# hermanjakobsen/robotic-ultrasound-imaging

Hardware: AMD Instinct MI355X
Metric: env-steps/sec (whole node) at 4096 envs/GPU, random-action rollout (higher is better)
Workload: dtype f32

## Files before the change

### robotic-ultrasound-imaging_amd/csrc/usim_step16.h

```cpp
#pragma once
#include <type_traits>

namespace usim {

template <int N, class F>
DI void static_for(F&& f) {
    if constexpr (N > 0) { static_for<N - 1>(f); f(std::integral_constant<int, N - 1>{}); }
}

template <int CTRL>
DI float dpp0(float v) { return __int_as_float(__builtin_amdgcn_update_dpp(0, __float_as_int(v), CTRL, 0xf, 0xf, true)); }
template <int G> DI int glane() { return (int)(threadIdx.x & (G - 1)); }
template <int G, int K> DI float rbc(float v) {
    if constexpr (G == 16) return dpp0<0x150 + K>(v);
    else {
        const int iv = __float_as_int(v);
        const int t = __builtin_amdgcn_update_dpp(iv, iv, 0x150 + K, 0xf, 0x3, false);
        return __int_as_float(__builtin_amdgcn_update_dpp(t, iv, 0x150 + 8 + K, 0xf, 0xc, false));
    }
}
template <int G, int D> DI float rshr0(float v) {
    const float t = dpp0<0x110 + D>(v);
    if constexpr (G == 16) return t; else return (glane<G>() < D) ? 0.f : t;
}
template <int G, int D> DI float rshl0(float v) {
    const float t = dpp0<0x100 + D>(v);
    if constexpr (G == 16) return t; else return (glane<G>() >= G - D) ? 0.f : t;
}
template <int G, int D> DI float rshr(float v, float fill) {
    const float t = __int_as_float(__builtin_amdgcn_update_dpp(__float_as_int(fill), __float_as_int(v), 0x110 + D, 0xf, 0xf, false));
    if constexpr (G == 16) return t; else return (glane<G>() < D) ? fill : t;
}
template <int K> DI float qbc(float v) { return dpp0<K * 0x55>(v); }
template <int G, int K> DI f3 rbc3(f3 v) { return mk(rbc<G, K>(v.x), rbc<G, K>(v.y), rbc<G, K>(v.z)); }
template <int G> DI float prefix_sum(float v) { v += rshr0<G, 1>(v); v += rshr0<G, 2>(v); v += rshr0<G, 4>(v); return v; }
template <int G> DI float suffix_sum(float v) { v += rshl0<G, 1>(v); v += rshl0<G, 2>(v); v += rshl0<G, 4>(v); return v; }
template <int G> DI f3 prefix_sum(f3 v) { return mk(prefix_sum<G>(v.x), prefix_sum<G>(v.y), prefix_sum<G>(v.z)); }
template <int G> DI f3 suffix_sum(f3 v) { return mk(suffix_sum<G>(v.x), suffix_sum<G>(v.y), suffix_sum<G>(v.z)); }

constexpr int TASK_LANE[6] = {0, 1, 2, 4, 5, 6};

#define USIM_DPP_BC(K) " row_newbcast:" #K " row_mask:0xf bank_mask:0xf\n\t"
#define USIM_DPP_LO(K) " row_newbcast:" #K " row_mask:0xf bank_mask:0x3\n\t"
DI float row_times_joint7(const float* A, float v) {
    float s;
    asm("s_nop 1\n\t"
        "v_mul_f32_dpp %0, %1, %2" USIM_DPP_BC(0) "v_fmac_f32_dpp %0, %1, %3" USIM_DPP_BC(1) "v_fmac_f32_dpp %0, %1, %4" USIM_DPP_BC(2)
        "v_fmac_f32_dpp %0, %1, %5" USIM_DPP_BC(3) "v_fmac_f32_dpp %0, %1, %6" USIM_DPP_BC(4) "v_fmac_f32_dpp %0, %1, %7" USIM_DPP_BC(5)
        "v_fmac_f32_dpp %0, %1, %8" USIM_DPP_BC(6)
        : "=&v"(s) : "v"(v), "v"(A[0]), "v"(A[1]), "v"(A[2]), "v"(A[3]), "v"(A[4]), "v"(A[5]), "v"(A[6]));
    return s;
}
DI float row_times_joint7_g8(const float* A, float v) {
    float s;
    asm("s_nop 1\n\t"
        "v_mul_f32_dpp %0, %1, %2 row_newbcast:0 row_mask:0xf bank_mask:0x3\n\t"  "v_mul_f32_dpp %0, %1, %2 row_newbcast:8 row_mask:0xf bank_mask:0xc\n\t"
        "v_fmac_f32_dpp %0, %1, %3 row_newbcast:1 row_mask:0xf bank_mask:0x3\n\t" "v_fmac_f32_dpp %0, %1, %3 row_newbcast:9 row_mask:0xf bank_mask:0xc\n\t"
        "v_fmac_f32_dpp %0, %1, %4 row_newbcast:2 row_mask:0xf bank_mask:0x3\n\t" "v_fmac_f32_dpp %0, %1, %4 row_newbcast:10 row_mask:0xf bank_mask:0xc\n\t"
        "v_fmac_f32_dpp %0, %1, %5 row_newbcast:3 row_mask:0xf bank_mask:0x3\n\t" "v_fmac_f32_dpp %0, %1, %5 row_newbcast:11 row_mask:0xf bank_mask:0xc\n\t"
        "v_fmac_f32_dpp %0, %1, %6 row_newbcast:4 row_mask:0xf bank_mask:0x3\n\t" "v_fmac_f32_dpp %0, %1, %6 row_newbcast:12 row_mask:0xf bank_mask:0xc\n\t"
        "v_fmac_f32_dpp %0, %1, %7 row_newbcast:5 row_mask:0xf bank_mask:0x3\n\t" "v_fmac_f32_dpp %0, %1, %7 row_newbcast:13 row_mask:0xf bank_mask:0xc\n\t"
        "v_fmac_f32_dpp %0, %1, %8 row_newbcast:6 row_mask:0xf bank_mask:0x3\n\t" "v_fmac_f32_dpp %0, %1, %8 row_newbcast:14 row_mask:0xf bank_mask:0xc"
        : "=&v"(s) : "v"(v), "v"(A[0]), "v"(A[1]), "v"(A[2]), "v"(A[3]), "v"(A[4]), "v"(A[5]), "v"(A[6]));
    return s;
}
template <int G, int NJ_>
DI float row_times_joint(const float* A, float v) {
    static_assert(NJ_ == 7, "seven joint lanes");
    if constexpr (G == 16) return row_times_joint7(A, v); else return row_times_joint7_g8(A, v);
}
template <int G>
DI float col_times_task(const float* A, float t) {
    float s;
    if constexpr (G == 16) {
        asm("s_nop 1\n\t"
            "v_mul_f32_dpp %0, %1, %2" USIM_DPP_BC(0) "v_fmac_f32_dpp %0, %1, %3" USIM_DPP_BC(1) "v_fmac_f32_dpp %0, %1, %4" USIM_DPP_BC(2)
            "v_fmac_f32_dpp %0, %1, %5" USIM_DPP_BC(4) "v_fmac_f32_dpp %0, %1, %6" USIM_DPP_BC(5) "v_fmac_f32_dpp %0, %1, %7" USIM_DPP_BC(6)
            : "=&v"(s) : "v"(t), "v"(A[0]), "v"(A[1]), "v"(A[2]), "v"(A[3]), "v"(A[4]), "v"(A[5]));
    } else {
        asm("s_nop 1\n\t"
            "v_mul_f32_dpp %0, %1, %2 row_newbcast:0 row_mask:0xf bank_mask:0x3\n\t"  "v_mul_f32_dpp %0, %1, %2 row_newbcast:8 row_mask:0xf bank_mask:0xc\n\t"
            "v_fmac_f32_dpp %0, %1, %3 row_newbcast:1 row_mask:0xf bank_mask:0x3\n\t" "v_fmac_f32_dpp %0, %1, %3 row_newbcast:9 row_mask:0xf bank_mask:0xc\n\t"
            "v_fmac_f32_dpp %0, %1, %4 row_newbcast:2 row_mask:0xf bank_mask:0x3\n\t" "v_fmac_f32_dpp %0, %1, %4 row_newbcast:10 row_mask:0xf bank_mask:0xc\n\t"
            "v_fmac_f32_dpp %0, %1, %5 row_newbcast:4 row_mask:0xf bank_mask:0x3\n\t" "v_fmac_f32_dpp %0, %1, %5 row_newbcast:12 row_mask:0xf bank_mask:0xc\n\t"
            "v_fmac_f32_dpp %0, %1, %6 row_newbcast:5 row_mask:0xf bank_mask:0x3\n\t" "v_fmac_f32_dpp %0, %1, %6 row_newbcast:13 row_mask:0xf bank_mask:0xc\n\t"
            "v_fmac_f32_dpp %0, %1, %7 row_newbcast:6 row_mask:0xf bank_mask:0x3\n\t" "v_fmac_f32_dpp %0, %1, %7 row_newbcast:14 row_mask:0xf bank_mask:0xc"
            : "=&v"(s) : "v"(t), "v"(A[0]), "v"(A[1]), "v"(A[2]), "v"(A[3]), "v"(A[4]), "v"(A[5]));
    }
    return s;
}
template <int G, int K>
// ... 34 lines not shown
            "v_fmac_f32_dpp %0, %4, %10 row_newbcast:%13 row_mask:0xf bank_mask:0x3\n\t" "v_fmac_f32_dpp %0, %4, %10 row_newbcast:%14 row_mask:0xf bank_mask:0xc\n\t"
            "v_fmac_f32_dpp %0, %5, %11 row_newbcast:%13 row_mask:0xf bank_mask:0x3\n\t" "v_fmac_f32_dpp %0, %5, %11 row_newbcast:%14 row_mask:0xf bank_mask:0xc\n\t"
            "v_fmac_f32_dpp %0, %6, %12 row_newbcast:%13 row_mask:0xf bank_mask:0x3\n\t" "v_fmac_f32_dpp %0, %6, %12 row_newbcast:%14 row_mask:0xf bank_mask:0xc"
            : "=&v"(s) : "v"(z.x), "v"(z.y), "v"(z.z), "v"(vo.x), "v"(vo.y), "v"(vo.z), "v"(n.x), "v"(n.y), "v"(n.z), "v"(f.x), "v"(f.y), "v"(f.z), "n"(K), "n"(K + 8));
    }
    return s;
}

template <int G>
DI void fk16(const float* at, const float q, f3& X, f3& Y, f3& Z, f3& P) {
    float s, c;
    sincos_(q, s, c);
    const f3 f0 = mk(at[AT_RFIX], at[AT_RFIX + 1], at[AT_RFIX + 2]), f1 = mk(at[AT_RFIX + 3], at[AT_RFIX + 4], at[AT_RFIX + 5]);
    X = f0 * c + f1 * s; Y = f1 * c - f0 * s; Z = mk(at[AT_RFIX + 6], at[AT_RFIX + 7], at[AT_RFIX + 8]);
    P = mk(at[AT_LPOS], at[AT_LPOS + 1], at[AT_LPOS + 2]);
    static_for<3>([&](auto Dc) {
        constexpr int D = 1 << decltype(Dc)::value;
        const f3 LX = mk(rshr<G, D>(X.x, 1.f), rshr<G, D>(X.y, 0.f), rshr<G, D>(X.z, 0.f));
        const f3 LY = mk(rshr<G, D>(Y.x, 0.f), rshr<G, D>(Y.y, 1.f), rshr<G, D>(Y.z, 0.f));
        const f3 LZ = mk(rshr<G, D>(Z.x, 0.f), rshr<G, D>(Z.y, 0.f), rshr<G, D>(Z.z, 1.f));
        const f3 LP = mk(rshr0<G, D>(P.x), rshr0<G, D>(P.y), rshr0<G, D>(P.z));
        const f3 nX = LX * X.x + LY * X.y + LZ * X.z, nY = LX * Y.x + LY * Y.y + LZ * Y.z, nZ = LX * Z.x + LY * Z.y + LZ * Z.z;
        P = LP + LX * P.x + LY * P.y + LZ * P.z;
        X = nX; Y = nY; Z = nZ;
    });
}

DI void jacobian_rows(float* xl, const int gl, const float* Jc, float* Jr) {
    if (gl < 8) {
#pragma unroll
        for (int a = 0; a < 6; ++a) xl[a * 8 + gl] = Jc[a];
    }
    group_sync();
    int arow = (gl & 7) - ((gl & 4) ? 1 : 0);
    arow = arow > 5 ? 5 : arow;
    const float4 j0 = *reinterpret_cast<const float4*>(&xl[arow * 8]), j1 = *reinterpret_cast<const float4*>(&xl[arow * 8 + 4]);
    Jr[0] = j0.x; Jr[1] = j0.y; Jr[2] = j0.z; Jr[3] = j0.w; Jr[4] = j1.x; Jr[5] = j1.y; Jr[6] = j1.z; Jr[7] = j1.w;
}

template <int G>
DI float solve6_task(float* A, float b, const int gl) {
    static_for<6>([&](auto Kc) {
        constexpr int k = decltype(Kc)::value;
        constexpr int lk = TASK_LANE[k];
        const float g = (A[k] - (gl == lk ? 1.f : 0.f)) * rcp_(rbc<G, lk>(A[k]));
#pragma unroll
        for (int c = k + 1; c < 6; ++c) A[c] = fmaf(-g, rbc<G, lk>(A[c]), A[c]);
        b = fmaf(-g, rbc<G, lk>(b), b);
    });
    return b;
}

constexpr int X16_WORDS = 64;
constexpr int X16_RIGID_STRIDE = 84;

#ifndef USIM_WPR16
#define USIM_WPR16 4
#endif
#ifndef USIM_WPR8
#define USIM_WPR8 4
#endif
template <int G> constexpr int wpr() { return G == 16 ? USIM_WPR16 : USIM_WPR8; }
constexpr int MB_POSE = X16_WORDS;
constexpr int MB_OP = MB_POSE + 12;
constexpr int MB_W = MB_OP + 64;
constexpr int MB_Q = MB_W + 16;
constexpr int MB_GOAL = MB_Q + 100;
#ifndef USIM_DRAW_AHEAD
#define USIM_DRAW_AHEAD 1
#endif
constexpr bool DRAW_AHEAD = USIM_DRAW_AHEAD != 0;
#ifndef USIM_LIST_AHEAD
#define USIM_LIST_AHEAD 0
#endif
constexpr bool LIST_AHEAD = USIM_LIST_AHEAD != 0;
#ifndef USIM_LATTICE_AHEAD
#define USIM_LATTICE_AHEAD 1
#endif
constexpr bool LATTICE_AHEAD = USIM_LATTICE_AHEAD != 0;
#ifndef USIM_LATTICE_PRIO
#define USIM_LATTICE_PRIO 1
#endif
constexpr bool LATTICE_PRIO = USIM_LATTICE_PRIO != 0;
constexpr int MB_ACT = MB_GOAL + 12;
constexpr int X2_STRIDE = MB_ACT + (DRAW_AHEAD ? 8 : 0);
template <int G> constexpr int x2_base() { return TB_WORDS + (64 * wpr<G>() / G) * GE_STRIDE; }
static_assert(x2_base<16>() % 4 == 0 && x2_base<8>() % 4 == 0 && X2_STRIDE % 4 == 0 && MB_OP % 4 == 0 && MB_W % 4 == 0 && MB_ACT % 4 == 0, "mailbox block: 16-byte accesses");
static_assert((x2_base<8>() + 32 * X2_STRIDE) * 4 <= 160 * 1024, "split kernel with 8-lane groups: LDS of a CU");
#ifndef USIM_ARM_CULL16
#define USIM_ARM_CULL16 0
#endif
template <int G> constexpr int arm_cull_rounds() { return G == 16 ? USIM_ARM_CULL16 : 7; }
static_assert(!LATTICE_AHEAD || USIM_ARM_CULL16 == 0, "LATTICE_AHEAD: the arm wave must not need the integrated element positions (no broad-phase rounds on its side)");
template <int ROLE, int G, bool RES> constexpr bool lattice_ahead() { return LATTICE_AHEAD && ROLE != 0 && G == 16 && RES; }

#if defined(USIM_TSTAMP) || defined(USIM_TSTAMP_NOWAIT)
#define USIM_BAR() do { __syncthreads(); ++nbar; } while (0)
#else
#define USIM_BAR() __syncthreads()
#endif


constexpr int ARM_LDS_WORDS = A16_LANES * AT_STRIDE;
template <int TORSO, int ROLE, int G> constexpr int arm_lds_base();
template <int NE, class WR = NoWarm>
struct Carry {
    float dqj, qdj, q0j;
    Episode ep;
    float s[NE], sd[NE];
    WR wr;
};

template <int TORSO, int ROLE, int G> constexpr int arm_lds_base() {
    return ROLE != 0 ? x2_base<G>() + (64 * wpr<G>() / G) * X2_STRIDE : (TORSO ? SOFT16_LDS_WORDS : 16 * X16_RIGID_STRIDE);
}
static_assert((arm_lds_base<1, 1, 8>() + ARM_LDS_WORDS) * 4 <= 160 * 1024 && arm_lds_base<1, 1, 8>() % 4 == 0 && arm_lds_base<1, 1, 16>() % 4 == 0 && arm_lds_base<1, 0, 16>() % 4 == 0
              && arm_lds_base<0, 0, 16>() % 4 == 0, "arm table behind the LDS blocks of every 16-lane kernel");

template <int TORSO, int MODE, int ROLE, int NT, int G = 16, bool RES = false, class WR = NoWarm, bool AHEAD = false>
DI void step16_one(float* lds, const DevModel& M, const DevCfg& C, float* __restrict__ st, const int n, const int npad, const DevIO& io, const int flags, const long long rstep,
                   const bool first_pass, const int sub, const bool more, int& nbar, Carry<TORSO ? (N_TOP + G - 1) / G : 1, WR>& cy) {
    static_assert(!AHEAD || (ROLE == 1 && RES), "action drawn ahead: the arm wave of a resident split launch");
    constexpr bool WARM = !std::is_same<WR, NoWarm>::value;
    static_assert(!WARM || (TORSO == 1 && ROLE == 0) || (TORSO == 1 && MODE == 0), "warm start: the soft-torso kernels");
    constexpr int WPR = (ROLE != 0) ? wpr<G>() : 4;
    constexpr int EPW = 64 / G, EPB = WPR * EPW;
    static_assert(!RES || MODE == 0, "resident state: step launches only");
    constexpr int X2_BASE = x2_base<G>();
    constexpr unsigned GMASK = (G == 16) ? 0xffffu : 0xffu;
    static_assert(G == 16 || (TORSO == 1 && MODE == 0 && ROLE != 0), "8-lane groups: the split soft-torso step only");
    constexpr int NE = TORSO ? (N_TOP + G - 1) / G : 1;
    static_assert(ROLE == 0 || (TORSO == 1 && MODE == 0), "the split kernel is the soft-torso step");
    const int lane = threadIdx.x & 63, wave = (threadIdx.x >> 6) & (WPR - 1);
    constexpr bool LA = lattice_ahead<ROLE, G, RES>();
    constexpr bool RES_HERE = RES && (LA || !(ROLE == 2 && G == 16));
    const bool fresh = !RES_HERE || first_pass;
    const int gl = lane & (G - 1), ge = lane / G;
    const int gbase = lane - gl;
    const int eb = wave * EPW + ge;
    const bool auto_reset = (flags & LF_AUTO_RESET) != 0;
    unsigned long long* const dbg = io.dbg;
    const bool refill = (MODE == 1) && io.refill != 0;
    const int item_cnt = refill ? io.count[0] : 1;
    const int item_first = refill ? (int)blockIdx.x * EPB : 0;
    for (int item0 = item_first; item0 < item_cnt; item0 += refill ? (int)gridDim.x * EPB : 1) {
    int env = blockIdx.x * EPB + eb;
    bool valid = env < n;
    int item_ep = 0;
    if (refill) {
        valid = item0 + eb < item_cnt;
        const int2 it = valid ? io.items[item0 + eb] : make_int2(0, 0);
        env = it.x; item_ep = it.y;
    }
    const bool store = valid && gl == 0;
    const int ei = valid ? env : (refill ? 0 : n - 1);
#define LAT(w) st[(size_t)F_LAT * npad + (size_t)ei * LAT_ENV_WORDS + (w)]
#define EB(off) lds[TB_WORDS + eb * GE_STRIDE + (off)]
    float* const warm_rows = st + warm_index(io.bank_row0, npad, (size_t)ei);
    int mbo = X2_BASE + eb * X2_STRIDE;
    if constexpr (ROLE != 0) asm volatile("" : "+v"(mbo));
    float* const xl = (ROLE != 0) ? &lds[mbo]
                                  : (TORSO ? &lds[TB_WORDS + eb * GE_STRIDE + GE_WS] : &lds[eb * X16_RIGID_STRIDE]);
    static_assert(GE_WS + X16_WORDS <= GE_STRIDE, "transpose scratch overlays the wrench records");
    constexpr int GOAL_OFF = (ROLE != 0) ? MB_GOAL : (TORSO ? GE_CG + (MAXCAND + 1) * CG_WORDS - GE_WS : X16_WORDS);
    static_assert(GE_CG + (MAXCAND + 1) * CG_WORDS + 12 <= GE_STRIDE && X16_WORDS + 12 <= X16_RIGID_STRIDE, "room for the goal");
    float* const goal_lds = xl + GOAL_OFF;

    USIM_STAMP(dbg, 0);
    if constexpr (ROLE == 1) { if (dbg && blockIdx.x == 0 && threadIdx.x == 0) dbg[20] = __builtin_readcyclecounter(); }

    float at[AT_STRIDE];
    {
        constexpr int ARM_LDS = arm_lds_base<TORSO, ROLE, G>();
        const float4* ap = fresh ? reinterpret_cast<const float4*>(M.tables + TB_ARM + gl * AT_STRIDE) : reinterpret_cast<const float4*>(lds + ARM_LDS + gl * AT_STRIDE);
        if (fresh) {
#pragma unroll
            for (int v = 0; v < AT_STRIDE / 4; ++v) { const float4 x = ap[v]; at[4 * v] = x.x; at[4 * v + 1] = x.y; at[4 * v + 2] = x.z; at[4 * v + 3] = x.w; }
            if constexpr (RES && ROLE != 2) {
                if (lane < G) {
#pragma unroll
                    for (int v = 0; v < AT_STRIDE / 4; ++v) reinterpret_cast<float4*>(lds + ARM_LDS + gl * AT_STRIDE)[v] = make_float4(at[4 * v], at[4 * v + 1], at[4 * v + 2], at[4 * v + 3]);
                }
            }
        } else {
            const float4* lp = reinterpret_cast<const float4*>(lds + ARM_LDS + gl * AT_STRIDE);
#pragma unroll
            for (int v = 0; v < AT_STRIDE / 4; ++v) { const float4 x = lp[v]; at[4 * v] = x.x; at[4 * v + 1] = x.y; at[4 * v + 2] = x.z; at[4 * v + 3] = x.w; }
        }
    }
    const float* const sp = st + scalar_index(0, (size_t)ei);
    const bool jlane = at[AT_JOINT] != 0.f;
    const int jl = jlane ? gl : NJ - 1;
    float &dqj = cy.dqj, &qdj = cy.qdj, &q0j = cy.q0j;
    Episode& E = cy.ep;
    f3 &ts = E.ts, &te = E.te;
    float &u0 = E.u0, &vbar = E.vbar, &fzbar = E.fzbar, &fzprev = E.fzprev, &dfz = E.dfz, &kst = E.kst, &kdmp = E.kdmp, &mu = E.mu, &epret = E.epret;
    int &t = E.t, &touched = E.touched, &episode = E.episode, &status = E.status;
    float (&s_pre)[NE] = cy.s, (&sd_pre)[NE] = cy.sd;
    if (fresh) {
        dqj = sp[F_Q + jl]; qdj = sp[F_QD + jl]; q0j = sp[F_Q0 + jl];
        float sv[20];
        {
            const float4* s4 = reinterpret_cast<const float4*>(sp + 20);
#pragma unroll
            for (int v = 0; v < 5; ++v) { const float4 x = s4[v]; sv[4 * v] = x.x; sv[4 * v + 1] = x.y; sv[4 * v + 2] = x.z; sv[4 * v + 3] = x.w; }
        }
#define SV(f) sv[(f) - 20]
        ts = mk(SV(F_TS), SV(F_TS + 1), SV(F_TS + 2)); te = mk(SV(F_TE), SV(F_TE + 1), SV(F_TE + 2));
        u0 = SV(F_U0); vbar = SV(F_VBAR); fzbar = SV(F_FZBAR); fzprev = SV(F_FZPREV); dfz = SV(F_DFZ);
        kst = SV(F_KST); kdmp = SV(F_KDMP); mu = SV(F_MU); epret = SV(F_EPRET);
        t = __float_as_int(SV(F_T)); touched = __float_as_int(SV(F_TOUCH)); episode = __float_as_int(SV(F_EPISODE)); status = __float_as_int(SV(F_STATUS));
#undef SV
#pragma unroll
        for (int i = 0; i < NE; ++i) {
            const int e = gl + i * G;
            s_pre[i] = 0.f; sd_pre[i] = 0.f;
            if (TORSO && MODE == 0 && ROLE != 1 && e < N_TOP) { s_pre[i] = LAT(LAT_S + e); sd_pre[i] = LAT(LAT_SD + e); }
            if (TORSO && MODE == 0 && ROLE == 1 && !LA && e < N_TOP) s_pre[i] = LAT(LAT_S + e);
        }
        if constexpr (WARM && MODE == 0 && ROLE != 1) warm_load(warm_rows, gl, cy.wr);
    } else if constexpr (RES && ROLE == 1 && !LA) {
#pragma unroll
        for (int i = 0; i < NE; ++i) { const int e = gl + i * G; s_pre[i] = (e < N_TOP) ? EB(GE_S + e) : 0.f; }
    } else if constexpr (RES && ROLE == 2 && !LA) {
        const float4 nx = *reinterpret_cast<const float4*>(&lds[mbo + MB_W]);
        if (nx.w != 0.f) {
            kst = nx.x; kdmp = nx.y; mu = nx.z; t = 0;
#pragma unroll
            for (int i = 0; i < NE; ++i) { s_pre[i] = 0.f; sd_pre[i] = 0.f; }
            warm_clear(cy.wr);
        }
    }
    if (!jlane) { dqj = 0.f; qdj = 0.f; q0j = 0.f; }
    float qj = q0j + dqj;
    if (TORSO != 0 && item0 == item_first && first_pass) {
        const float4* src = reinterpret_cast<const float4*>(M.tables);
        float4* dst = reinterpret_cast<float4*>(lds);
        constexpr int NV = TB_WORDS / 4, PER = (NV + NT - 1) / NT;
        float4 tmp[PER];
        int tix = threadIdx.x;
        asm volatile("" : "+v"(tix));
#pragma unroll
        for (int i = 0; i < PER; ++i) { int idx = tix + i * NT; tmp[i] = (idx < NV) ? src[idx] : make_float4(0, 0, 0, 0); }
#pragma unroll
        for (int i = 0; i < PER; ++i) { int idx = tix + i * NT; if (idx < NV) dst[idx] = tmp[i]; }
        USIM_BAR();
    }
    USIM_STAMP(dbg, 1);

    if (MODE == 0 && sub == 0) t += 1;
    const bool last_sub = sub == C.substeps - 1;
    const int tphys = (MODE == 0) ? (t - 1) * C.substeps + sub : 0;
    const float dt = C.dt, inv_h = rcp_((float)C.horizon);
#if defined(USIM_TSTAMP) || defined(USIM_TSTAMP_NOWAIT)
#define RSTAMP(k) do { if (dbg && blockIdx.x == 0 && (threadIdx.x & (64 * WPR - 1)) == 0) dbg[(ROLE == 2 ? 30 : 20) + (k)] = __builtin_readcyclecounter(); } while (0)
#else
#define RSTAMP(k) do { } while (0)
#endif
#define XSTAMP(k) RSTAMP(20 + (k))
    if constexpr (ROLE == 2) {
        RSTAMP(0);
        if constexpr (LA && LATTICE_PRIO) __builtin_amdgcn_s_setprio(1);
        float* const mb = &lds[mbo];
        const int* tb_shell = reinterpret_cast<const int*>(lds + TB_SHELL);
        float dz, vz, az;
        torso_motion(C, tphys, dz, vz, az);
        if constexpr (LA) {
            if (first_pass) {
#pragma unroll
                for (int i = 0; i < NE; ++i) { const int e = gl + i * G; if (e < N_TOP) EB(GE_S + e) = s_pre[i]; }
            }
        }
        lattice_rhs<G, NE>(lds, eb, gl, M, az, kst, kdmp, true, s_pre, sd_pre);
        lattice_solve<G>(lds, eb, gl, gbase);
        RSTAMP(1);
        USIM_BAR();
        RSTAMP(2);
        if constexpr (LA && LATTICE_PRIO) __builtin_amdgcn_s_setprio(0);
        if constexpr (LA) {
            if (!first_pass) {
                const float4 nx = *reinterpret_cast<const float4*>(&mb[MB_W]);
                const bool began = nx.w != 0.f;
                if (__any(began)) {
                    if (began) {
                        kst = nx.x; kdmp = nx.y; mu = nx.z; t = 0;
                        if (sub == 0) t += 1;
#pragma unroll
                        for (int i = 0; i < NE; ++i) { const int e = gl + i * G; s_pre[i] = 0.f; sd_pre[i] = 0.f; if (e < N_TOP) EB(GE_S + e) = 0.f; }
                        warm_clear(cy.wr);
                    }
                    torso_motion(C, (t - 1) * C.substeps + sub, dz, vz, az);
                    lattice_rhs<G, NE>(lds, eb, gl, M, az, kst, kdmp, true, s_pre, sd_pre);
                    lattice_solve<G>(lds, eb, gl, gbase);
                }
            }
        }
        const f3 xs = mk(mb[MB_POSE], mb[MB_POSE + 1], mb[MB_POSE + 2]), sy = mk(mb[MB_POSE + 3], mb[MB_POSE + 4], mb[MB_POSE + 5]),
                 sz = mk(mb[MB_POSE + 6], mb[MB_POSE + 7], mb[MB_POSE + 8]);
        const f3 sxc = cross(sy, sz);
        int nq = __float_as_int(mb[MB_POSE + 10]);
#pragma unroll
        for (int i = arm_cull_rounds<G>(); i < NE; ++i) {
            const int eraw = i * G + gl, e = eraw < N_TOP ? eraw : N_TOP - 1;
            const bool cand = (eraw < N_TOP) && collide_cull(lds, e, M, C, s_pre[i], dz, xs, sxc, sz);
            const unsigned gm = (unsigned)(__ballot(cand) >> gbase) & GMASK;
            mb[MB_Q + (cand ? nq + __popc(gm & ((1u << gl) - 1u)) : 99)] = __int_as_float(e);
            nq += __popc(gm);
        }
        group_sync();
#if defined(USIM_TSTAMP) || defined(USIM_TSTAMP_NOWAIT)
        if (dbg && blockIdx.x == 0 && wave == 0 && gl == 0) dbg[54 + ge] = 1ull + (unsigned long long)nq;
#endif
        int nc = 0;
        collide_queue<G>(lds, mb + MB_Q, nq, &EB(GE_CG), gl, gbase, M, C, &EB(GE_S), dz, xs, sxc, sy, sz, nc);
        constexpr bool EARLY = G == 8;
        ContactRows P;
        constexpr bool LIST_EARLY = EARLY || (G == 16 && LIST_AHEAD);
        int nc_early = nc, overflow_early = 0, ncmax_early = 0, cel_early[MAXC];
        if constexpr (LIST_EARLY) {
            contact_overflow<G>(lds, eb, gl, gbase, nc_early);
            if (nc_early > MAXC) { overflow_early = 1; nc_early = MAXC; }
            group_sync();
            if constexpr (G == 16) {
                const int m01 = max(__builtin_amdgcn_readlane(nc_early, 0), __builtin_amdgcn_readlane(nc_early, 16));
                const int m23 = max(__builtin_amdgcn_readlane(nc_early, 32), __builtin_amdgcn_readlane(nc_early, 48));
                ncmax_early = max(m01, m23);
            } else {
#pragma unroll
                for (int k = MAXC; k >= 1; --k) if (ncmax_early == 0 && __any(nc_early >= k)) ncmax_early = k;
            }
#pragma unroll
            for (int k = 0; k < MAXC; ++k) cel_early[k] = (k < nc_early) ? __float_as_int(EB(GE_CG + k * CG_WORDS + 6)) : 0;
            if constexpr (EARLY) { if (ncmax_early > 0) contact_rows<G>(lds, eb, gl, M, C, nc_early, cel_early, vz, P); }
        }
        RSTAMP(3);
        USIM_BAR();
        RSTAMP(4);
        if constexpr (LA && LATTICE_PRIO) __builtin_amdgcn_s_setprio(1);
        if constexpr (!LIST_EARLY) contact_overflow<G>(lds, eb, gl, gbase, nc);
        int overflow = 0;
        if (nc > MAXC) { overflow = 1; nc = MAXC; }
        if constexpr (!LIST_EARLY) group_sync();
        XSTAMP(0);
        int ncmax = 0;
        if constexpr (LIST_EARLY) { nc = nc_early; overflow = overflow_early; ncmax = ncmax_early; }
        else {
#pragma unroll
            for (int k = MAXC; k >= 1; --k) if (ncmax == 0 && __any(nc >= k)) ncmax = k;
        }
        XSTAMP(1);
        float gf[MAXC], W[6] = {0, 0, 0, 0, 0, 0};
        int cel[MAXC];
#pragma unroll
        for (int k = 0; k < MAXC; ++k) { const int ek = __float_as_int(EB(GE_CG + k * CG_WORDS + 6)); gf[k] = 0.f; cel[k] = LIST_EARLY ? cel_early[k] : ((k < nc) ? ek : 0); }
        if (ncmax > 0) {
            float alpha[6], vs[6], Lp[21];
#pragma unroll
            for (int a = 0; a < 6; ++a) {
                alpha[a] = mb[MB_OP + 48 + a]; vs[a] = mb[MB_OP + 54 + a];
#pragma unroll
                for (int b = 0; b <= a; ++b) Lp[PK(a, b)] = mb[MB_OP + a * 8 + b];
            }
            XSTAMP(2);
            contact_solve<G, EARLY, true>(lds, eb, gl, M, C, nc, ncmax, cel, Lp, alpha, vs, mu, vz, P, W, gf, dbg, cy.wr);
            XSTAMP(3);
        } else warm_clear(cy.wr);
        if (gl == 0) {
            *reinterpret_cast<float4*>(&mb[MB_W]) = make_float4(W[0], W[1], W[2], W[3]);
            *reinterpret_cast<float4*>(&mb[MB_W + 4]) = make_float4(W[4], W[5], __int_as_float(nc), __int_as_float(overflow));
#pragma unroll
            for (int k = 0; k < MAXC; ++k) { const int sh = tb_shell[cel[k]]; mb[MB_W + 8 + k] = __int_as_float((k < nc) ? sh : -1); }
        }
        RSTAMP(5);
        USIM_BAR();
        RSTAMP(6);
#if defined(USIM_TSTAMP) || defined(USIM_TSTAMP_NOWAIT)
        if (more && dbg && blockIdx.x == 0 && (threadIdx.x & (64 * WPR - 1)) == 0) dbg[62] = __builtin_readcyclecounter();
#endif
        {
            float acc_e[NE];
#pragma unroll
            for (int i = 0; i < NE; ++i) { const int e = gl + i * G; acc_e[i] = (e < N_TOP) ? EB(GE_A + e) : 0.f; }
#pragma unroll
            for (int k = 0; k < MAXC; ++k) {
#pragma unroll
                for (int i = 0; i < NE; ++i) {
                    const int e = (gl + i * G < N_TOP) ? gl + i * G : N_TOP - 1;
                    acc_e[i] = fmaf(lds[TB_LINV + e * LROW + cel[k]], gf[k], acc_e[i]);
                }
            }
#pragma unroll
            for (int i = 0; i < NE; ++i) {
                const int e = gl + i * G;
                if (e >= N_TOP) continue;
                const float sdn = sd_pre[i] + dt * acc_e[i];
                const float sn = s_pre[i] + dt * sdn;
                if (valid) { LAT(LAT_SD + e) = sdn; LAT(LAT_S + e) = sn; }
                if constexpr (RES) { sd_pre[i] = sdn; s_pre[i] = sn; EB(GE_S + e) = sn; }
            }
            if constexpr (WARM) { if (valid) warm_store(warm_rows, gl, cy.wr); }
        }
        RSTAMP(7);
        if (!LA || !more) USIM_BAR();
        RSTAMP(8);
        return;
    }
    const int comp = gl & 3;
    const bool blk = (gl & 4) != 0;
    const bool is_task = (gl < 8) && comp != 3;
    auto pick = [&](f3 v) { return comp == 0 ? v.x : (comp == 1 ? v.y : v.z); };

    bool need = false;
    int ep_t = episode;
    if constexpr (MODE == 1) {
        need = refill ? valid : (io.mask ? io.mask[ei] != 0 : true);
        if (!__any(need)) continue;
        ep_t = refill ? item_ep : episode + 1;
        if (!refill) episode = ep_t;
        const uint32_t gid = (uint32_t)(C.env_offset + ei);
        const u4 r = philox(gid, (uint32_t)ep_t, (uint32_t)(gl < 3 ? gl : 2), 0u, C.key0, C.key1);
        const float ra = __uint_as_float(r.a), rb = __uint_as_float(r.b), rc = __uint_as_float(r.c), rd = __uint_as_float(r.d);
        u4 A, B, Cc;
        A.a = __float_as_uint(rbc<G, 0>(ra)); A.b = __float_as_uint(rbc<G, 0>(rb)); A.c = __float_as_uint(rbc<G, 0>(rc)); A.d = __float_as_uint(rbc<G, 0>(rd));
        B.a = __float_as_uint(rbc<G, 1>(ra)); B.b = __float_as_uint(rbc<G, 1>(rb)); B.c = __float_as_uint(rbc<G, 1>(rc)); B.d = __float_as_uint(rbc<G, 1>(rd));
        Cc.a = __float_as_uint(rbc<G, 2>(ra)); Cc.b = __float_as_uint(rbc<G, 2>(rb)); Cc.c = __float_as_uint(rbc<G, 2>(rc)); Cc.d = __float_as_uint(rbc<G, 2>(rd));
        const float tz = M.torso[2] + M.base[2] + C.top_off;
        f3 noise = mk(0, 0, 0);
        kst = C.stiffness; kdmp = C.damping;
        if (io.reset_params) {
            const float* p = io.reset_params + (size_t)ei * 13;
            ts = mk(p[0], p[1], p[2]); te = mk(p[3], p[4], p[5]); u0 = p[6]; noise = mk(p[7], p[8], p[9]);
            kst = p[10]; kdmp = p[11]; mu = p[12];
        } else {
            if (C.det_traj) { ts = mk(0.062f, -0.020f, 0.896f); te = mk(-0.032f, -0.075f, 0.896f); }
            else {
                const float tx = M.torso[0] + M.base[0], ty = M.torso[1] + M.base[1];
                const float xs0 = -0.15f + tx + 0.03f, xstep = (0.15f + tx - xs0) / 49.f;
                const float ys0 = -C.y_range + ty, ystep = 2.f * C.y_range / 49.f;
                ts = mk(xs0 + (float)urange(A.a, 50u) * xstep, ys0 + (float)urange(A.b, 50u) * ystep, tz);
                te = mk(xs0 + (float)urange(A.c, 50u) * xstep, ys0 + (float)urange(A.d, 50u) * ystep, tz);
            }
            u0 = u01(B.a);
            if (C.rand_pos) {
                const float r1 = sqrtf(-2.f * logf(u01_open(B.b))), th1 = 2.f * PI_F * u01(B.c);
                const float r2 = sqrtf(-2.f * logf(u01_open(B.d))), th2 = 2.f * PI_F * u01(Cc.a);
                noise = mk(r1 * cosf(th1) * 0.0025f, r1 * sinf(th1) * 0.0025f, r2 * cosf(th2) * 0.010f);
            }
            if (C.rand_solref) { kst = 1300.f + (float)urange(Cc.b, 300u); kdmp = 17.f + (float)urange(Cc.c, 24u); }
            float pf = C.probe_fric;
            if (C.rand_fric) pf *= 0.5f + 1.5f * u01(Cc.d);
            mu = fmaxf(pf, C.elem_fric);
            if (C.probe_geoms == 2 && !C.pair) mu = 0.5f * (mu + fmaxf(C.probe_fric2, C.elem_fric));
        }
        const float uu = clampf(u0, 0.f, 1.f);
        const f3 tp0 = ts + (te - ts) * uu;
        const f3 target = mk(tp0.x + noise.x + M.ikb[0] - M.base[0], tp0.y + noise.y + M.ikb[1] - M.base[1], tp0.z + noise.z + M.ikb[2] - M.base[2]);
        const f3 gx = mk(M.grot[0], M.grot[3], M.grot[6]), gy = mk(M.grot[1], M.grot[4], M.grot[7]), gz = mk(M.grot[2], M.grot[5], M.grot[8]);
        qj = jlane ? at[AT_INITQ] : 0.f;
        for (int it = 0; it < C.ik_iters; ++it) {
            f3 X, Y, Z, P;
            fk16<G>(at, qj, X, Y, Z, P);
            const f3 sx = rbc3<G, 7>(X), sy = rbc3<G, 7>(Y), sz = rbc3<G, 7>(Z), xs = rbc3<G, 7>(P);
            const f3 eo = (cross(sx, gx) + cross(sy, gy) + cross(sz, gz)) * 0.5f;
            const f3 ep = target - xs;
            const float e = is_task ? (blk ? pick(eo) : pick(ep)) : 0.f;
            const f3 jv = cross(Z, xs - P);
            const float Jc[6] = {jlane ? jv.x : 0.f, jlane ? jv.y : 0.f, jlane ? jv.z : 0.f, jlane ? Z.x : 0.f, jlane ? Z.y : 0.f, jlane ? Z.z : 0.f};
            float Jr[8];
            jacobian_rows(xl, gl, Jc, Jr);
            float A6[6];
            static_for<6>([&](auto Bc) {
                constexpr int b = decltype(Bc)::value;
                float sacc = 0.f;
                static_for<NJ>([&](auto Jn) { constexpr int j = decltype(Jn)::value; sacc = fmaf(Jr[j], rbc<G, TASK_LANE[b]>(Jr[j]), sacc); });
                A6[b] = is_task ? sacc + ((gl == TASK_LANE[b]) ? 1e-6f : 0.f) : 0.f;
            });
            const float y = solve6_task<G>(A6, e, gl);
            const float dq = col_times_task<G>(Jc, y);
            qj = jlane ? qj + dq : 0.f;
            group_sync();
        }
        q0j = qj; qdj = 0.f; dqj = 0.f;
        episode_begin(E, 0);
// ... 436 lines not shown
            if (refill) {
                if (valid && need) {
                    const int sl = ep_t & (BANK_DEPTH - 1);
                    if (jlane) BK(sl, BQ0 + gl) = qj;
                    if (gl == 0) {
                        BK(sl, BTS) = ts.x; BK(sl, BTS + 1) = ts.y; BK(sl, BTS + 2) = ts.z; BK(sl, BTE) = te.x; BK(sl, BTE + 1) = te.y; BK(sl, BTE + 2) = te.z;
                        BK(sl, BU0) = u0; BK(sl, BKST) = kst; BK(sl, BKDMP) = kdmp; BK(sl, BMU) = mu; BK(sl, BFZ) = fzbar;
#pragma unroll
                        for (int a = 0; a < OBS_DIM; ++a) BK(sl, BOBS + a) = obs[a];
                        BKI(sl, BSTATUS) = overflow ? 1 : 0;
                    }
                }
            } else if (store && io.obs && need) {
#pragma unroll
                for (int a = 0; a < OBS_DIM; ++a) io.obs[(size_t)ei * OBS_DIM + a] = obs[a];
            }
        } else if (last_sub) {
        const bool contact = ncon > 0;
        if (contact) touched = 1;
        const float force_rew = contact ? force_e : 0.f, dforce_rew = contact ? dforce_e : 0.f;
        float reward = pos_rew + ori_rew + vel_rew + force_rew + dforce_rew;
        done = t >= C.horizon;
        const float hvn = sqrt_(dot(hv, hv));
        vbar += (hvn - vbar) * rcp_((float)t);
        const float fz = W[2];
        dfz = (fz - fzprev) * rcp_(C.dt_ctrl);
        fzprev = fz;
        fzbar = 0.1f * fz + 0.9f * fzbar;
        const bool jviol = (qj < at[AT_QMIN] + 0.1f) || (qj > at[AT_QMAX] - 0.1f);
        const unsigned jany = (unsigned)(__ballot(jviol) >> gbase) & GMASK;
        if (C.early_term) {
            const bool term = (jany != 0u) || (pos_err_norm > 1.0f) || (contact && ori_err > 0.10f) || (touched && !contact);
            done = done || term;
        }
        epret += reward;
        if (io.log && valid) {
            float* L = io.log + (size_t)ei * LOG_WIDTH;
            if (jlane) L[26 + gl] = qj;
            if (gl == 0) {
                const float upn = clampf((float)t * inv_h + u0, 0.f, 1.f);
                const f3 tpn = ts + (te - ts) * upn;
                L[0] = xw.x; L[1] = xw.y; L[2] = xw.z; L[3] = tpn.x; L[4] = tpn.y; L[5] = tpn.z;
                L[6] = hv.x; L[7] = hv.y; L[8] = hv.z; L[9] = 0.04f; L[10] = vbar;
                L[11] = qe[0]; L[12] = qe[1]; L[13] = qe[2]; L[14] = qe[3];
                L[15] = M.gquat[0]; L[16] = M.gquat[1]; L[17] = M.gquat[2]; L[18] = M.gquat[3];
                L[19] = ori_err * 5.0f;
                L[20] = fz; L[21] = 5.0f; L[22] = fzbar; L[23] = dfz; L[24] = 0.f; L[25] = contact ? 1.f : 0.f;
                L[40] = (float)(t - 1) * inv_h * 100.f;
                L[41] = pos_rew; L[42] = ori_rew; L[43] = vel_rew; L[44] = force_rew; L[45] = dforce_rew;
            }
        }
        if (overflow) status |= 1;
        {
            const float chk = rbc<G, 7>(prefix_sum<G>(fabsf(qj) + 1e-3f * fabsf(qdj)));
            if (!(chk < 1.0e3f)) { status |= 4; done = true; epret -= reward; reward = 0.f; if (!(epret == epret)) epret = 0.f; }
        }
        if (store) {
            io.rew[ei] = reward;
            if (io.status_out) io.status_out[ei] = status;
            io.done[ei] = done ? 1 : 0;
            if (io.contacts) {
                io.contacts[(size_t)ei * (1 + MAXC)] = ncon;
#pragma unroll
                for (int k = 0; k < MAXC; ++k) io.contacts[(size_t)ei * (1 + MAXC) + 1 + k] = con_shell[k];
            }
            if (done) {
                if (io.term_obs) {
#pragma unroll
                    for (int a = 0; a < OBS_DIM; ++a) io.term_obs[(size_t)ei * OBS_DIM + a] = obs[a];
                }
                if (io.ep_ret) io.ep_ret[ei] = epret;
                if (io.ep_len) io.ep_len[ei] = t;
            }
        }
        need = done && auto_reset;
        if (store && io.obs && !need) {
#pragma unroll
            for (int a = 0; a < OBS_DIM; ++a) io.obs[(size_t)ei * OBS_DIM + a] = obs[a];
        }
        }
    }

    if constexpr (ROLE == 1) { RSTAMP(7); if (!LA || !more) USIM_BAR(); RSTAMP(8); }
    if (MODE == 0 && need) {
        episode += 1;
        const int sl = episode & (BANK_DEPTH - 1);
        qj = jlane ? BK(sl, BQ0 + jl) : 0.f; q0j = qj; qdj = 0.f; dqj = 0.f;
        ts = mk(BK(sl, BTS), BK(sl, BTS + 1), BK(sl, BTS + 2)); te = mk(BK(sl, BTE), BK(sl, BTE + 1), BK(sl, BTE + 2));
        u0 = BK(sl, BU0); kst = BK(sl, BKST); kdmp = BK(sl, BKDMP); mu = BK(sl, BMU); fzbar = BK(sl, BFZ);
        episode_begin(E, BKI(sl, BSTATUS));
        if (store && io.obs) {
#pragma unroll
            for (int a = 0; a < OBS_DIM; ++a) io.obs[(size_t)ei * OBS_DIM + a] = BK(sl, BOBS + a);
        }
        const bool zero_here = !LA || !more;
        if (TORSO && valid && zero_here) for (int e = gl; e < N_TOP; e += G) { LAT(LAT_S + e) = 0.f; LAT(LAT_SD + e) = 0.f; }
        if constexpr (WARM) {
            if (valid && zero_here) warm_rows_clear<G>(warm_rows, gl);
            warm_clear(cy.wr);
        }
        if constexpr (RES && TORSO != 0) {
#pragma unroll
            for (int i = 0; i < NE; ++i) {
                s_pre[i] = 0.f; sd_pre[i] = 0.f;
                if (ROLE == 1 && !LA && gl + i * G < N_TOP) EB(GE_S + gl + i * G) = 0.f;
            }
        }
        if (store) order_refill(io, env, episode);
    }
    if constexpr (RES && ROLE == 1) {
        if (gl == 0) *reinterpret_cast<float4*>(&xl[MB_W]) = make_float4(kst, kdmp, mu, (MODE == 0 && need) ? 1.f : 0.f);
    }
    USIM_STAMP(dbg, 15);

    if (valid && (MODE == 0 || (need && !refill))) {
        float* const so = st + scalar_index(0, (size_t)ei);
        if (jlane) {
            so[F_Q + gl] = dqj; so[F_QD + gl] = qdj;
            if (need) so[F_Q0 + gl] = q0j;
        }
        if (gl == 0) {
            float4* s4 = reinterpret_cast<float4*>(so);
            if (need) {
                so[F_TS] = ts.x; so[F_TS + 1] = ts.y; so[F_TS + 2] = ts.z;
                s4[6] = make_float4(te.x, te.y, te.z, u0);
            }
            s4[7] = make_float4(vbar, fzbar, fzprev, dfz);
            s4[8] = make_float4(kst, kdmp, mu, __int_as_float(t));
            s4[9] = make_float4(__int_as_float(touched), __int_as_float(episode), epret, __int_as_float(status));
        }
    }
    if (refill) group_sync();
    }
    if (MODE == 1 && refill) work_list_close(io);
    USIM_STAMP(dbg, 16);
    if constexpr (ROLE == 1) RSTAMP(9);
#undef RSTAMP
#undef XSTAMP
#undef LAT
#undef EB
}

template <int TORSO, int MODE, int ROLE, int NT, bool MULTI = false, int G = 16, class WR = NoWarm, bool ACTS = false>
DI void step16_body(float* lds, const DevModel& M, const DevCfg& C, float* __restrict__ st, const int n, const int npad, const DevIO& io0, const int flags, const long long rstep) {
    const int S = (MULTI && MODE == 0 && C.substeps > 1) ? C.substeps : 1;
    const int nsub = (MULTI && MODE == 0) ? (io0.nsub > 1 ? io0.nsub : 1) * S : 1;
    DevIO io = io0;
    int nbar = 0;
    Carry<TORSO ? (N_TOP + G - 1) / G : 1, WR> cy;
    int sub = 0;
    long long cstep = rstep;
    for (int ks = 0; ks < nsub; ++ks) {
        constexpr bool AHEAD = DRAW_AHEAD && ROLE == 1 && MULTI && MODE == 0 && !ACTS;
        step16_one<TORSO, MODE, ROLE, NT, G, MULTI && MODE == 0, WR, AHEAD>(lds, M, C, st, n, npad, io, flags, cstep, ks == 0, sub, ks + 1 < nsub, nbar, cy);
        const bool ctrl_done = sub == S - 1;
        if (ctrl_done) { sub = 0; ++cstep; } else ++sub;
        if (ks + 1 < nsub) {
            constexpr bool LA = lattice_ahead<ROLE, G, MULTI && MODE == 0>();
            if constexpr (!LA) {
                __threadfence_block();
                if constexpr (ROLE != 0) USIM_BAR();
            }
            if (io0.block && ctrl_done) advance_rollout_block(io, (size_t)n, C.adim);
            if constexpr (ACTS) { if (ctrl_done) io.act += (size_t)n * C.adim; }
        }
    }
#if defined(USIM_TSTAMP) || defined(USIM_TSTAMP_NOWAIT)
    if (ROLE != 0 && io0.dbg && blockIdx.x == 0 && (threadIdx.x & (64 * wpr<G>() - 1)) == 0) io0.dbg[ROLE == 1 ? 46 : 47] = (unsigned long long)nbar;
#endif
}

template <int TORSO, int OCC, int MODE, bool MULTI = false, bool WARM = false>
__global__ __launch_bounds__(256) __attribute__((amdgpu_waves_per_eu(OCC, OCC))) void usim_step16_kernel(const DevModel M, const DevCfg C, float* __restrict__ st, int n, int npad,
                                                                                                          const DevIO io, int flags, long long rstep) {
    extern __shared__ __attribute__((aligned(16))) float lds[];
    step16_body<TORSO, MODE, 0, 256, MULTI, 16, typename std::conditional<WARM, WarmOf<16>::type, NoWarm>::type>(lds, M, C, st, n, npad, io, flags, rstep);
}

template <int TORSO, int OCC, bool WARM = false>
__global__ __launch_bounds__(256) __attribute__((amdgpu_waves_per_eu(OCC, OCC))) void usim_step16_acts_kernel(const DevModel M, const DevCfg C, float* __restrict__ st, int n, int npad,
                                                                                                               const DevIO io, int flags, long long rstep) {
    extern __shared__ __attribute__((aligned(16))) float lds[];
    step16_body<TORSO, 0, 0, 256, true, 16, typename std::conditional<WARM, WarmOf<16>::type, NoWarm>::type, true>(lds, M, C, st, n, npad, io, flags, rstep);
}

template <bool MULTI, int G = 16, bool WARM = false>
__global__ __launch_bounds__(128 * wpr<G>()) __attribute__((amdgpu_waves_per_eu(2, 2))) void usim_step32_kernel(const DevModel* __restrict__ Mp, const DevCfg* __restrict__ Cp, float* __restrict__ st, int n, int npad,
                                                                                                                  const DevIO io, int flags, long long rstep) {
    extern __shared__ __attribute__((aligned(16))) float lds[];
    const DevModel& M = *Mp; const DevCfg& C = *Cp;
    constexpr int NT = 128 * wpr<G>();
    typedef typename std::conditional<WARM, typename WarmOf<G>::type, NoWarm>::type WR;
    if (threadIdx.x < NT / 2) step16_body<1, 0, 1, NT, MULTI, G, WR>(lds, M, C, st, n, npad, io, flags, rstep);
    else step16_body<1, 0, 2, NT, MULTI, G, WR>(lds, M, C, st, n, npad, io, flags, rstep);
}

template <int G = 16, bool WARM = false>
__global__ __launch_bounds__(128 * wpr<G>()) __attribute__((amdgpu_waves_per_eu(2, 2))) void usim_step32_acts_kernel(const DevModel* __restrict__ Mp, const DevCfg* __restrict__ Cp, float* __restrict__ st, int n, int npad,
                                                                                                                       const DevIO io, int flags, long long rstep) {
    extern __shared__ __attribute__((aligned(16))) float lds[];
    const DevModel& M = *Mp; const DevCfg& C = *Cp;
    constexpr int NT = 128 * wpr<G>();
    typedef typename std::conditional<WARM, typename WarmOf<G>::type, NoWarm>::type WR;
    if (threadIdx.x < NT / 2) step16_body<1, 0, 1, NT, true, G, WR, true>(lds, M, C, st, n, npad, io, flags, rstep);
    else step16_body<1, 0, 2, NT, true, G, WR, true>(lds, M, C, st, n, npad, io, flags, rstep);
}
// ... 3 lines not shown
```

Baseline: 243.5 million.

## Pin carried registers to avoid drain waits and optionally defer state writeback

Adds empty inline-asm register pins on carried state and staged table loads in the lattice-ahead resident split kernel, so the compiler stops inserting memory-counter drain waits before values are used. The episode-reset block is wrapped in a wave-uniform __any(need) branch so waves with no resets skip it. An optional mode, off by default, writes the lattice, warm rows and scalar state back to memory only on the last resident step, and then always writes the reset fields. The pins may raise VGPR pressure, and the deferred writeback depends on nothing reading that state between steps.

```diff
diff --git a/robotic-ultrasound-imaging_amd/csrc/usim_step16.h b/robotic-ultrasound-imaging_amd/csrc/usim_step16.h
--- a/robotic-ultrasound-imaging_amd/csrc/usim_step16.h
+++ b/robotic-ultrasound-imaging_amd/csrc/usim_step16.h
@@ -7,6 +7,12 @@
 DI void static_for(F&& f) {
     if constexpr (N > 0) { static_for<N - 1>(f); f(std::integral_constant<int, N - 1>{}); }
 }
+
+DI void pin_v(float& x) { asm volatile("" : "+v"(x)); }
+DI void pin_v(int& x) { asm volatile("" : "+v"(x)); }
+DI void pin_v(f3& v) { pin_v(v.x); pin_v(v.y); pin_v(v.z); }
+DI void pin_v(NoWarm&) {}
+DI void pin_v(WarmRec<float>& r) { pin_v(r.el); pin_v(r.f[0]); pin_v(r.f[1]); pin_v(r.f[2]); pin_v(r.lam); }
 
 template <int CTRL>
 DI float dpp0(float v) { return __int_as_float(__builtin_amdgcn_update_dpp(0, __float_as_int(v), CTRL, 0xf, 0xf, true)); }
@@ -207,6 +213,14 @@
 #define USIM_LATTICE_PRIO 1
 #endif
 constexpr bool LATTICE_PRIO = USIM_LATTICE_PRIO != 0;
+#ifndef USIM_WRITEBACK_LAST
+#define USIM_WRITEBACK_LAST 0
+#endif
+constexpr bool WRITEBACK_LAST = USIM_WRITEBACK_LAST != 0;
+#ifndef USIM_NO_DRAIN_WAITS
+#define USIM_NO_DRAIN_WAITS 1
+#endif
+constexpr bool NO_DRAIN_WAITS = USIM_NO_DRAIN_WAITS != 0;
 constexpr int MB_ACT = MB_GOAL + 12;
 constexpr int X2_STRIDE = MB_ACT + (DRAW_AHEAD ? 8 : 0);
 template <int G> constexpr int x2_base() { return TB_WORDS + (64 * wpr<G>() / G) * GE_STRIDE; }
@@ -259,6 +273,8 @@
     const int lane = threadIdx.x & 63, wave = (threadIdx.x >> 6) & (WPR - 1);
     constexpr bool LA = lattice_ahead<ROLE, G, RES>();
     constexpr bool RES_HERE = RES && (LA || !(ROLE == 2 && G == 16));
+    constexpr bool WBL = LA && WRITEBACK_LAST, NDW = LA && NO_DRAIN_WAITS;
+    const bool wb = !WBL || !more;
     const bool fresh = !RES_HERE || first_pass;
     const int gl = lane & (G - 1), ge = lane / G;
     const int gbase = lane - gl;
@@ -344,6 +360,18 @@
             if (TORSO && MODE == 0 && ROLE == 1 && !LA && e < N_TOP) s_pre[i] = LAT(LAT_S + e);
         }
         if constexpr (WARM && MODE == 0 && ROLE != 1) warm_load(warm_rows, gl, cy.wr);
+        if constexpr (NDW) {
+            if constexpr (ROLE == 1) {
+                pin_v(dqj); pin_v(qdj); pin_v(q0j);
+                pin_v(ts); pin_v(te); pin_v(u0); pin_v(vbar); pin_v(fzbar); pin_v(fzprev); pin_v(dfz); pin_v(kst); pin_v(kdmp); pin_v(mu); pin_v(epret);
+                pin_v(t); pin_v(touched); pin_v(episode); pin_v(status);
+            } else {
+                pin_v(kst); pin_v(kdmp); pin_v(mu); pin_v(t);
+#pragma unroll
+                for (int i = 0; i < NE; ++i) { pin_v(s_pre[i]); pin_v(sd_pre[i]); }
+                pin_v(cy.wr);
+            }
+        }
     } else if constexpr (RES && ROLE == 1 && !LA) {
 #pragma unroll
         for (int i = 0; i < NE; ++i) { const int e = gl + i * G; s_pre[i] = (e < N_TOP) ? EB(GE_S + e) : 0.f; }
@@ -369,6 +397,10 @@
         for (int i = 0; i < PER; ++i) { int idx = tix + i * NT; tmp[i] = (idx < NV) ? src[idx] : make_float4(0, 0, 0, 0); }
 #pragma unroll
         for (int i = 0; i < PER; ++i) { int idx = tix + i * NT; if (idx < NV) dst[idx] = tmp[i]; }
+        if constexpr (NDW) {
+#pragma unroll
+            for (int i = 0; i < PER; ++i) { pin_v(tmp[i].x); pin_v(tmp[i].y); pin_v(tmp[i].z); pin_v(tmp[i].w); }
+        }
         USIM_BAR();
     }
     USIM_STAMP(dbg, 1);
@@ -520,10 +552,10 @@
                 if (e >= N_TOP) continue;
                 const float sdn = sd_pre[i] + dt * acc_e[i];
                 const float sn = s_pre[i] + dt * sdn;
-                if (valid) { LAT(LAT_SD + e) = sdn; LAT(LAT_S + e) = sn; }
+                if (valid && wb) { LAT(LAT_SD + e) = sdn; LAT(LAT_S + e) = sn; }
                 if constexpr (RES) { sd_pre[i] = sdn; s_pre[i] = sn; EB(GE_S + e) = sn; }
             }
-            if constexpr (WARM) { if (valid) warm_store(warm_rows, gl, cy.wr); }
+            if constexpr (WARM) { if (valid && wb) warm_store(warm_rows, gl, cy.wr); }
         }
         RSTAMP(7);
         if (!LA || !more) USIM_BAR();
@@ -1126,6 +1158,7 @@
     }
 
     if constexpr (ROLE == 1) { RSTAMP(7); if (!LA || !more) USIM_BAR(); RSTAMP(8); }
+    if (MODE == 0 && (!NDW || __any(need))) {
     if (MODE == 0 && need) {
         episode += 1;
         const int sl = episode & (BANK_DEPTH - 1);
@@ -1152,20 +1185,22 @@
         }
         if (store) order_refill(io, env, episode);
     }
+    if constexpr (NDW) { pin_v(q0j); pin_v(ts); pin_v(te); pin_v(u0); pin_v(kst); pin_v(kdmp); pin_v(mu); pin_v(fzbar); pin_v(status); }
+    }
     if constexpr (RES && ROLE == 1) {
         if (gl == 0) *reinterpret_cast<float4*>(&xl[MB_W]) = make_float4(kst, kdmp, mu, (MODE == 0 && need) ? 1.f : 0.f);
     }
     USIM_STAMP(dbg, 15);
 
-    if (valid && (MODE == 0 || (need && !refill))) {
+    if (valid && wb && (MODE == 0 || (need && !refill))) {
         float* const so = st + scalar_index(0, (size_t)ei);
         if (jlane) {
             so[F_Q + gl] = dqj; so[F_QD + gl] = qdj;
-            if (need) so[F_Q0 + gl] = q0j;
+            if (WBL || need) so[F_Q0 + gl] = q0j;
         }
         if (gl == 0) {
             float4* s4 = reinterpret_cast<float4*>(so);
-            if (need) {
+            if (WBL || need) {
                 so[F_TS] = ts.x; so[F_TS + 1] = ts.y; so[F_TS + 2] = ts.z;
                 s4[6] = make_float4(te.x, te.y, te.z, u0);
             }
```

Result: no change. 245.0 million (median of 6 runs) (+0.6%).
